# rednote-hilab/dots.ocr

Hardware: AMD Instinct MI355X
Metric: pages/sec, dots.ocr 1.7B bf16, A4@200dpi page batch (preprocess + ViT + prefill + 1024-token greedy decode + detokenise) (higher is better)
Workload: dtype bf16; 1 GPU; a4: 8 pages/GPU of 1654x2339 px -> 19824 patches, 5200 prompt tokens/page, max_new_tokens=1024, EOS disabled; pages_per_gpu=8, parallelism=dp1, decode_rows_in_flight=64

## Files before the change

dots_ocr_amd/csrc/engine.hip:

```cpp
#include <hip/hip_runtime.h>
#include <hip/hip_fp16.h>

#include <algorithm>
#include <cmath>
#include <cstdarg>
#include <cstddef>
#include <cstdio>
#include <cstdlib>
#include <cstring>
#include <string>
#include <unordered_map>
#include <vector>

#include "common.h"
#include "decode_layout.h"
#include "dots_ocr_hip.h"
#include "kernels.h"

namespace {

thread_local std::string g_create_error;

struct Tensor {
    bf16_t* p = nullptr;
// ... 1683 lines not shown
int dots_set_decode_plan(DotsEngine* e, int plan) {
    if (!e) return DOTS_E_INVALID;
    if (plan < 0 || plan > 5 || (plan & 6) == 6)
        return e->fail(DOTS_E_INVALID, "decode plan must be 0 (by stream) or 1 (partition plan on every step), + 2 (streaming attention) or + 4 (per-split attention)");
    const int part = plan & 1, stream = (plan & 2) ? 1 : (plan & 4) ? 0 : -1;
    if (part != e->force_part || stream != e->attn_stream) {
        e->force_part = part;
        e->attn_stream = stream;
        drop_step_graphs(e);
    }
    return DOTS_OK;
}

int dots_tower_tail(DotsEngine* e, int set, int* now) {
    if (!e) return DOTS_E_INVALID;
    if (set < -2 || set > e->cfg.v_layers) return e->fail(DOTS_E_INVALID, "tower tail must be -2 (query), -1 (adaptive) or 0 .. v_layers");
    if (set >= -1) e->tail_fixed = set;
    if (now) *now = e->tail_now;
    return DOTS_OK;
}

int dots_set_gemm_plan(DotsEngine* e, int plan) {
    if (!e) return DOTS_E_INVALID;
    if (plan < 0 || plan > 1) return e->fail(DOTS_E_INVALID, "gemm plan must be 0 (8-wave ping-pong) or 1 (one wave per SIMD)");
    gemm_set_plan(plan);
    return DOTS_OK;
}

int dots_get_logits(DotsEngine* e, float* out) {
    if (!e || !out) return DOTS_E_INVALID;
    if (e->B < 1) return e->fail(DOTS_E_STATE, "no prefilled batch");
    CK(hipSetDevice(e->device));
    CK(hipMemcpyAsync(out, e->d_logits, (size_t)e->B * e->cfg.vocab_size * 4, hipMemcpyDeviceToHost, e->stream));
    CK(hipStreamSynchronize(e->stream));
    return DOTS_OK;
}

int dots_set_next_tokens(DotsEngine* e, const int32_t* tokens, int B) {
    if (!e || !tokens || B != e->B) return e ? e->fail(DOTS_E_INVALID, "bad set_next_tokens arguments") : DOTS_E_INVALID;
    CK(hipSetDevice(e->device));
    CK(hipMemcpyAsync(e->cur_tokens, tokens, B * 4, hipMemcpyHostToDevice, e->stream));
    CK(hipStreamSynchronize(e->stream));
    return DOTS_OK;
}

int dots_get_last_tokens(DotsEngine* e, int32_t* out) {
    if (!e || !out) return DOTS_E_INVALID;
// ... 490 lines not shown
```

dots_ocr_amd/csrc/gemm.hip:

```cpp
#include <cstdlib>
#include <utility>

#include "common.h"
#include "kernels.h"

namespace {

constexpr int BM = 128, BN = 128, BK = 64;
constexpr int TILE_BYTES = 128 * 128;
#ifndef GEMM_GROUP_M
#define GEMM_GROUP_M 8
#endif
constexpr int GROUP_M = GEMM_GROUP_M;

DEVI float gelu_erf(float x) { return 0.5f * x * (1.0f + erff(x * 0.70710678118654752440f)); }
#ifdef GEMM_EXACT_SILU
DEVI float silu(float x) { return x / (1.0f + __expf(-x)); }
#else
DEVI float silu(float x) {
    const float d = 1.0f + __expf(fminf(-x, 80.f));
    const float r = __builtin_amdgcn_rcpf(d);
    const float q = x * r;
    return __builtin_fmaf(__builtin_fmaf(-q, d, x), r, q);
}
#endif

template <int EPI, int FN, int FM = 2>
DEVI void gemm_epilogue(const f32x16 (&acc)[FN][FM], const bf16_t* __restrict__ bias, const float* __restrict__ colscale, const bf16_t* R,
                        void* Cout, int M, int ldc, int nw0, int mw0, int l31, int hi, const float* __restrict__ rowscale = nullptr) {
#pragma unroll
    for (int fm = 0; fm < FM; ++fm) {
        const int m = mw0 + fm * 32 + l31;
        if (m >= M) continue;
        const float rs = rowscale ? rowscale[m] : 1.f;
        if constexpr (EPI == EPI_SWIGLU) {
            bf16_t* C = reinterpret_cast<bf16_t*>(Cout);
// ... 425 lines not shown
    const int gcol = SW ? ((l & 7) >> 2) * 64 + (l & 3) * 8 : (l & 15) * 8;
    u32x4 b0 = {0, 0, 0, 0}, b1 = {0, 0, 0, 0};
    f32x4 s00 = {1.f, 1.f, 1.f, 1.f}, s01 = s00, s10 = s00, s11 = s00;
    if (bias) {
        b0 = *reinterpret_cast<const u32x4*>(bias + nw0 + gcol);
        if (SW) b1 = *reinterpret_cast<const u32x4*>(bias + nw0 + gcol + 32);
    }
    if (colscale) {
        s00 = *reinterpret_cast<const f32x4*>(colscale + nw0 + gcol);
        s01 = *reinterpret_cast<const f32x4*>(colscale + nw0 + gcol + 4);
        if (SW) {
            s10 = *reinterpret_cast<const f32x4*>(colscale + nw0 + gcol + 32);
            s11 = *reinterpret_cast<const f32x4*>(colscale + nw0 + gcol + 36);
        }
    }
#pragma unroll
    for (int e = 0; e < 4; ++e) {
        cc.sc0[e] = s00[e]; cc.sc0[4 + e] = s01[e]; cc.sc1[e] = s10[e]; cc.sc1[4 + e] = s11[e];
        cc.bi0[2 * e] = lo_bf(b0[e]); cc.bi0[2 * e + 1] = hi_bf(b0[e]);
        cc.bi1[2 * e] = lo_bf(b1[e]); cc.bi1[2 * e + 1] = hi_bf(b1[e]);
    }
}

template <int EPI, bool FULL>
DEVI void w4_epilogue_lds(const f32x16 (&acc)[4][4], const W4Cols& cc, bool has_cols, const bf16_t* R,
                          bf16_t* __restrict__ C, int M, int ldc, int nw0, int mw0, int l, char* stage2) {
    const int hi = l >> 5, l31 = l & 31;
    constexpr bool SW = EPI == EPI_SWIGLU;
    constexpr int ITS = SW ? 4 : 8, RPI = SW ? 8 : 4;
    const int rrow = SW ? (l >> 3) : (l >> 4);
    const int gcol = SW ? ((l & 7) >> 2) * 64 + (l & 3) * 8 : (l & 15) * 8;
    const int col = SW ? nw0 / 2 + ((l & 7) >> 2) * 32 + (l & 3) * 8 : nw0 + gcol;
    u32x4 rr[2][8];
    auto load_r = [&](int fm, u32x4 (&dst)[8]) {
        if constexpr (EPI == EPI_RESIDUAL) {
#pragma unroll
            for (int it = 0; it < ITS; ++it) {
                const int m = FULL ? mw0 + fm * 32 + it * RPI + rrow : min(mw0 + fm * 32 + it * RPI + rrow, M - 1);
                dst[it] = *reinterpret_cast<const u32x4*>(R + (size_t)m * ldc + col);
            }
        }
    };
#ifdef W4_OLD_SWZ
    auto swz = [](int row) { return (row & 15) << 1; };
#else
    auto swz = [](int row) { return ((row & 15) << 1) ^ (row & 1) ^ ((row & 2) << 2); };
#endif
    const int wslot = swz(l31);
    char* const wrow = stage2 + l31 * 512;
#define W4_PUT(FM, IMG)                                                                                                   \
    _Pragma("unroll") for (int fn = 0; fn < 4; ++fn) _Pragma("unroll") for (int rq = 0; rq < 4; ++rq) {                     \
        const f32x4 v = {acc[fn][FM][4 * rq], acc[fn][FM][4 * rq + 1], acc[fn][FM][4 * rq + 2], acc[fn][FM][4 * rq + 3]};   \
        *reinterpret_cast<f32x4*>(wrow + (IMG) * 16384 + (((fn * 8 + rq * 2 + hi) ^ wslot) << 4)) = v;                      \
    }
    load_r(0, rr[0]);
    W4_PUT(0, 0)
#pragma unroll
    for (int fm = 0; fm < 4; ++fm) {
        if (fm + 1 < 4) {
            load_r(fm + 1, rr[(fm + 1) & 1]);
            if (fm == 0) { W4_PUT(1, 1) } else if (fm == 1) { W4_PUT(2, 0) } else { W4_PUT(3, 1) }
        }
        __builtin_amdgcn_sched_barrier(0);
        const char* img = stage2 + (fm & 1) * 16384;
        f32x4 a[ITS][SW ? 4 : 2];
#pragma unroll
        for (int it = 0; it < ITS; ++it) {
            const int row = it * RPI + rrow;
            const int sw = swz(row);
            const char* rp = img + row * 512;
            const int s0 = gcol >> 2;
            a[it][0] = *reinterpret_cast<const f32x4*>(rp + ((s0 ^ sw) << 4));
            a[it][1] = *reinterpret_cast<const f32x4*>(rp + (((s0 + 1) ^ sw) << 4));
            if constexpr (SW) {
                a[it][2] = *reinterpret_cast<const f32x4*>(rp + (((s0 + 8) ^ sw) << 4));
                a[it][3] = *reinterpret_cast<const f32x4*>(rp + (((s0 + 9) ^ sw) << 4));
            }
// ... 41 lines not shown

DEVI void w4_load_cols_rope(W4Cols& cc, const bf16_t* __restrict__ bias, const float* __restrict__ colscale, int nw0, int l) {
    const int gcol = (l & 15) * 8, pcol = gcol ^ 64;
    u32x4 b0 = {0, 0, 0, 0}, b1 = {0, 0, 0, 0};
    f32x4 s00 = {1.f, 1.f, 1.f, 1.f}, s01 = s00, s10 = s00, s11 = s00;
    if (bias) {
        b0 = *reinterpret_cast<const u32x4*>(bias + nw0 + gcol);
        b1 = *reinterpret_cast<const u32x4*>(bias + nw0 + pcol);
    }
    if (colscale) {
        s00 = *reinterpret_cast<const f32x4*>(colscale + nw0 + gcol);
        s01 = *reinterpret_cast<const f32x4*>(colscale + nw0 + gcol + 4);
        s10 = *reinterpret_cast<const f32x4*>(colscale + nw0 + pcol);
        s11 = *reinterpret_cast<const f32x4*>(colscale + nw0 + pcol + 4);
    }
#pragma unroll
    for (int e = 0; e < 4; ++e) {
        cc.sc0[e] = s00[e]; cc.sc0[4 + e] = s01[e]; cc.sc1[e] = s10[e]; cc.sc1[4 + e] = s11[e];
        cc.bi0[2 * e] = lo_bf(b0[e]); cc.bi0[2 * e + 1] = hi_bf(b0[e]);
        cc.bi1[2 * e] = lo_bf(b1[e]); cc.bi1[2 * e + 1] = hi_bf(b1[e]);
    }
}

template <bool FULL>
DEVI void w4_epilogue_qkrope(const f32x16 (&acc)[4][4], const W4Cols& cc, bool has_cols, const float2* __restrict__ cs, bf16_t* __restrict__ dst,
                             int M, int mw0, int l, char* stage2) {
    const int hi = l >> 5, l31 = l & 31;
    const int rrow = l >> 4, gcol = (l & 15) * 8;
    const bool lo_half = (l & 8) == 0;
    const float2* const tab = cs + (gcol & 63);
    auto swz = [](int row) { return ((row & 15) << 1) ^ (row & 1) ^ ((row & 2) << 2); };
    const int wslot = swz(l31);
    char* const wrow = stage2 + l31 * 512;
#define W4_PUT(FM, IMG)                                                                                                   \
    _Pragma("unroll") for (int fn = 0; fn < 4; ++fn) _Pragma("unroll") for (int rq = 0; rq < 4; ++rq) {                     \
        const f32x4 v = {acc[fn][FM][4 * rq], acc[fn][FM][4 * rq + 1], acc[fn][FM][4 * rq + 2], acc[fn][FM][4 * rq + 3]};   \
        *reinterpret_cast<f32x4*>(wrow + (IMG) * 16384 + (((fn * 8 + rq * 2 + hi) ^ wslot) << 4)) = v;                      \
    }
    f32x4 tb[2][2][4];
    auto load_t = [&](int qb, f32x4 (&d)[2][4]) {
#pragma unroll
        for (int it = 0; it < 2; ++it) {
            const int m = FULL ? mw0 + qb * 8 + it * 4 + rrow : min(mw0 + qb * 8 + it * 4 + rrow, M - 1);
            const f32x4* tp = reinterpret_cast<const f32x4*>(tab + (size_t)m * 64);
#pragma unroll
            for (int c = 0; c < 4; ++c) d[it][c] = tp[c];
        }
    };
    load_t(0, tb[0]);
    W4_PUT(0, 0)
#pragma unroll
    for (int qb = 0; qb < 16; ++qb) {
        const int fm = qb >> 2;
        if (qb + 1 < 16) load_t(qb + 1, tb[(qb + 1) & 1]);
        if ((qb & 3) == 0 && fm + 1 < 4) {
            if (fm == 0) { W4_PUT(1, 1) } else if (fm == 1) { W4_PUT(2, 0) } else { W4_PUT(3, 1) }
        }
        __builtin_amdgcn_sched_barrier(0);
        const char* img = stage2 + (fm & 1) * 16384;
        f32x4 a[2][4];
#pragma unroll
// ... 18 lines not shown
                for (int e = 0; e < 8; ++e) { o[e] = o[e] * cc.sc0[e] + cc.bi0[e]; u[e] = u[e] * cc.sc1[e] + cc.bi1[e]; }
            }
            uint32_t pk[4];
#pragma unroll
            for (int e = 0; e < 4; ++e) {
                const uint32_t ow = pack_bf2(o[2 * e], o[2 * e + 1]), uw = pack_bf2(u[2 * e], u[2 * e + 1]);
                const float x0 = lo_bf(ow), x1 = hi_bf(ow), y0 = lo_bf(uw), y1 = hi_bf(uw);
                const f32x4 t4 = tb[qb & 1][it][e];
                const float f0 = lo_half ? x0 : y0, g0 = lo_half ? t4[0] : t4[1], m0 = lo_half ? y0 : x0, n0_ = lo_half ? t4[1] : t4[0];
                const float p0 = m0 * n0_, p1 = y1 * t4[3];
                const float r0 = __builtin_fmaf(f0, g0, lo_half ? -p0 : p0), r1 = __builtin_fmaf(x1, t4[2], lo_half ? -p1 : p1);
                pk[e] = pack_bf2(r0, r1);
            }
            if (FULL || m < M) *reinterpret_cast<u32x4*>(dst + (size_t)m * 128 + gcol) = u32x4{pk[0], pk[1], pk[2], pk[3]};
        }
        __builtin_amdgcn_sched_barrier(0);
    }
#undef W4_PUT
}

template <int... I, class F> DEVI void gemm_static_for_impl(std::integer_sequence<int, I...>, F&& f) { (f(std::integral_constant<int, I>{}), ...); }
template <int N, class F> DEVI void gemm_static_for(F&& f) { gemm_static_for_impl(std::make_integer_sequence<int, N>{}, f); }

template <int EPI>
DEVI void gemm_bf16_w4_body(
    const bf16_t* __restrict__ A, const bf16_t* __restrict__ W, const bf16_t* __restrict__ bias,
    const float* __restrict__ colscale, const bf16_t* R, void* Cout, int M, int N, int K, int lda, int ldc, int m_tiles, int n_tiles, int group_m, const QkRope& rope) {
    extern __shared__ __attribute__((aligned(16))) char smem2[];
    (void)rope;

    const int tid = threadIdx.x;
    const int l = tid & 63;
    const int w = __builtin_amdgcn_readfirstlane(tid >> 6);
    const int hi = l >> 5, l31 = l & 31;

    int bid = xcd_remap(blockIdx.x, m_tiles * n_tiles);
    const int per_group = group_m * n_tiles;
    const int g = bid / per_group;
    const int first_m = g * group_m;
    const int gsz = min(m_tiles - first_m, group_m);
    const int in_grp = bid - g * per_group;
    const int tm = first_m + in_grp % gsz;
    const int tn = in_grp / gsz;
    const int m0 = tm * BM2, n0 = tn * BN2;

    const int prow = 8 * w + (l >> 3);
    const int chunk = ((l & 7) ^ ((4 * w + (l >> 4)) & 7)) << 4;
    const int w_src = prow * (K * 2) + chunk;
    int x_src[8];
#pragma unroll
    for (int i = 0; i < 8; ++i) x_src[i] = (min(m0 + prow + 32 * i, M - 1) - m0) * (lda * 2) + chunk;
    const __amdgpu_buffer_rsrc_t rw = __builtin_amdgcn_make_buffer_rsrc((void*)(W + (size_t)n0 * K), 0, 0x7ffffff0, 0x00020000);
    const __amdgpu_buffer_rsrc_t rx = __builtin_amdgcn_make_buffer_rsrc((void*)(A + (size_t)m0 * lda), 0, 0x7ffffff0, 0x00020000);
    const int w_step = 32 * K * 2;
    auto dma_w = [&](int t, int slot, int i) {
        __builtin_amdgcn_raw_ptr_buffer_load_lds(rw, (__attribute__((address_space(3))) void*)(smem2 + slot * W4_UNIT + (w + 4 * i) * 1024), 16, w_src,
                                                 t * 128 + i * w_step, 0, 0);
    };
    auto dma_x = [&](int t, int slot, int i) {
        __builtin_amdgcn_raw_ptr_buffer_load_lds(rx, (__attribute__((address_space(3))) void*)(smem2 + slot * W4_UNIT + (w + 4 * i) * 1024), 16, x_src[i],
                                                 t * 128, 0, 0);
    };

    const int wn = w >> 1, wm = w & 1;
    const int rsw = (l31 >> 1) & 7;
    const int lane_sw = ((hi ^ (rsw & 1)) << 4) | ((rsw >> 1) << 5);
    const int lds0 = (int)(uintptr_t)(__attribute__((address_space(3))) char*)smem2;
    const int a_lane = lds0 + (wn * 128 + l31) * 128 + lane_sw;
    const int b_lane = lds0 + (wm * 128 + l31) * 128 + lane_sw;
    auto frag = [&](int base, int ks, int f) {
        return *reinterpret_cast<const __attribute__((address_space(3))) bf16x8*>((uintptr_t)(uint32_t)((base ^ (ks << 5)) + f * 4096));
    };

#ifdef W4_PROF
    const unsigned long long pt0 = __builtin_amdgcn_s_memtime(), pw0 = wall_clock64();
#endif
    W4Cols cols;
    if constexpr (EPI == EPI_QKROPE) w4_load_cols_rope(cols, bias, colscale, n0 + wn * 128, l);
    else if constexpr (EPI != EPI_F32) w4_load_cols<EPI == EPI_SWIGLU>(cols, bias, colscale, n0 + wn * 128, l);

    f32x16 acc[4][4];
#pragma unroll
    for (int i = 0; i < 4; ++i)
#pragma unroll
        for (int j = 0; j < 4; ++j)
#pragma unroll
            for (int r = 0; r < 16; ++r) acc[i][j][r] = 0.f;

    const int nt = K / BK;
#ifdef W4_STAGGER
    if (blockIdx.x < 256) {
        const int naps = ((blockIdx.x >> 3) & 7) * nt * W4_STAGGER / 8;
        for (int i = 0; i < naps; ++i) __builtin_amdgcn_s_sleep(8);
    }
#endif
#pragma unroll
    for (int u = 0; u < 4; ++u)
#pragma unroll
        for (int i = 0; i < 8; ++i) {
            if (u & 1) dma_x(u >> 1, u, i);
            else dma_w(u >> 1, u, i);
        }
    asm volatile("s_waitcnt vmcnt(16)" ::: "memory");
    __builtin_amdgcn_s_barrier();
    bf16x8 fa[2][4], fb[2][4];
#pragma unroll
    for (int f = 0; f < 4; ++f) { fa[0][f] = frag(a_lane, 0, f); fb[0][f] = frag(b_lane + W4_UNIT, 0, f); }
#ifdef W4_PROF
    const unsigned long long pt1 = __builtin_amdgcn_s_memtime(), pw1 = wall_clock64();
#endif

    auto tile_body = [&](auto mode_c, int t, int u0) {
        constexpr int MODE = decltype(mode_c)::value;
        const int s1 = u0 + 1 >= W4_RING ? u0 + 1 - W4_RING : u0 + 1, s2 = u0 + 2 >= W4_RING ? u0 + 2 - W4_RING : u0 + 2;
        const int s3 = u0 + 3 >= W4_RING ? u0 + 3 - W4_RING : u0 + 3, s4 = u0 + 4 >= W4_RING ? u0 + 4 - W4_RING : u0 + 4;
        const int aw = a_lane + u0 * W4_UNIT, ax = b_lane + s1 * W4_UNIT;
        const int awn = a_lane + s2 * W4_UNIT, axn = b_lane + s3 * W4_UNIT;
        gemm_static_for<64>([&acc, &fa, &fb, &frag, &dma_w, &dma_x, aw, ax, awn, axn, t, u0, s4](auto gc) {
            constexpr int gp = decltype(gc)::value;
            (void)acc; (void)t; (void)u0; (void)s4; (void)dma_w; (void)dma_x;
            constexpr int ks = gp >> 4, idx = gp & 15, fn = idx >> 2, fm = idx & 3, cur = ks & 1;
            if constexpr (gp == 48 && MODE < 2) {
                if constexpr (MODE == 0) asm volatile("s_waitcnt vmcnt(8) lgkmcnt(0)" ::: "memory");
                else asm volatile("s_waitcnt vmcnt(0) lgkmcnt(0)" ::: "memory");
                __builtin_amdgcn_s_barrier();
            }
            if constexpr (idx < 8 && (ks < 3 || MODE < 2)) {
                constexpr int f = idx & 3;
                if constexpr (ks < 3) {
                    if constexpr (idx < 4) fa[cur ^ 1][f] = frag(aw, ks + 1, f);
                    else fb[cur ^ 1][f] = frag(ax, ks + 1, f);
                } else {
                    if constexpr (idx < 4) fa[cur ^ 1][f] = frag(awn, 0, f);
                    else fb[cur ^ 1][f] = frag(axn, 0, f);
                }
            }
#ifndef W4_NO_DMA
            if constexpr (MODE == 0) {
                if constexpr (gp == 8 || gp == 11 || gp == 14 || gp == 24 || gp == 27 || gp == 30 || gp == 40 || gp == 43) {
                    constexpr int i = gp < 16 ? (gp - 8) / 3 : gp < 32 ? 3 + (gp - 24) / 3 : 6 + (gp - 40) / 3;
                    dma_w(t + 2, s4, i);
                }
                if constexpr (gp >= 56) dma_x(t + 2, u0, gp - 56);
            }
#endif
            asm volatile("v_mfma_f32_32x32x16_bf16 %[d], %[a], %[b], %[d]" : [d] "+a"(acc[fn][fm]) : [a] "v"(fa[cur][fn]), [b] "v"(fb[cur][fm]));
        });
    };
    int u0 = 0;
    for (int t = 0; t < nt - 2; ++t) {
        tile_body(std::integral_constant<int, 0>{}, t, u0);
        u0 = u0 + 2 >= W4_RING ? u0 + 2 - W4_RING : u0 + 2;
    }
    tile_body(std::integral_constant<int, 1>{}, nt - 2, u0);
    u0 = u0 + 2 >= W4_RING ? u0 + 2 - W4_RING : u0 + 2;
    tile_body(std::integral_constant<int, 2>{}, nt - 1, u0);

#ifdef W4_PROF
    const unsigned long long pt2 = __builtin_amdgcn_s_memtime(), pw2 = wall_clock64();
#endif
    __syncthreads();
#ifdef W4_NO_STORE
#pragma unroll
    for (int i = 0; i < 4; ++i)
#pragma unroll
        for (int j = 0; j < 4; ++j) asm volatile("" ::"a"(acc[i][j]));
    return;
#endif
#ifdef W4_OLD_EPILOGUE
    if constexpr (EPI == EPI_F32 || EPI == EPI_SWIGLU) {
        gemm_epilogue<EPI, 4, 4>(acc, bias, colscale, R, Cout, M, ldc, n0 + wn * 128, m0 + wm * 128, l31, hi);
    } else {
        gemm_epilogue_lds<EPI, 4>(acc, bias, colscale, R, reinterpret_cast<bf16_t*>(Cout), M, ldc, n0 + wn * 128, m0 + wm * 128, l, smem2 + w * 16384);
    }
#else
    if constexpr (EPI == EPI_QKROPE) {
        const int head = (n0 + wn * 128) >> 7;
        const bool full = m0 + wm * 128 + 128 <= M, has_cols = bias != nullptr || colscale != nullptr;
        if (head < rope.n_rope_heads) {
            bf16_t* dst = head < rope.Hq ? rope.q + (size_t)head * rope.T * 128 : rope.k + (size_t)(head - rope.Hq) * rope.T * 128;
            if (full) w4_epilogue_qkrope<true>(acc, cols, has_cols, rope.cs, dst, M, m0 + wm * 128, l, smem2 + w * 32768);
            else w4_epilogue_qkrope<false>(acc, cols, has_cols, rope.cs, dst, M, m0 + wm * 128, l, smem2 + w * 32768);
        } else if (full) {
            w4_epilogue_lds<EPI_NONE, true>(acc, cols, has_cols, R, reinterpret_cast<bf16_t*>(Cout), M, ldc, n0 + wn * 128, m0 + wm * 128, l, smem2 + w * 32768);
        } else {
            w4_epilogue_lds<EPI_NONE, false>(acc, cols, has_cols, R, reinterpret_cast<bf16_t*>(Cout), M, ldc, n0 + wn * 128, m0 + wm * 128, l, smem2 + w * 32768);
        }
    } else if constexpr (EPI == EPI_F32) {
        gemm_epilogue<EPI, 4, 4>(acc, bias, colscale, R, Cout, M, ldc, n0 + wn * 128, m0 + wm * 128, l31, hi);
    } else if (m0 + wm * 128 + 128 <= M) {
        w4_epilogue_lds<EPI, true>(acc, cols, bias != nullptr || colscale != nullptr, R, reinterpret_cast<bf16_t*>(Cout), M, ldc, n0 + wn * 128, m0 + wm * 128, l, smem2 + w * 32768);
    } else {
        w4_epilogue_lds<EPI, false>(acc, cols, bias != nullptr || colscale != nullptr, R, reinterpret_cast<bf16_t*>(Cout), M, ldc, n0 + wn * 128, m0 + wm * 128, l, smem2 + w * 32768);
    }
#endif
#ifdef W4_PROF
    const unsigned long long pt2b = __builtin_amdgcn_s_memtime();
    asm volatile("s_waitcnt vmcnt(0)" ::: "memory");
    const unsigned long long pt3 = __builtin_amdgcn_s_memtime(), pw3 = wall_clock64();
    if ((blockIdx.x == 1000 || blockIdx.x == 2001 || blockIdx.x == 3002) && tid == 0)
        printf("W4_PROF epi %d N %d K %d blk %d: prologue %llu cyc / %.2f us, main loop %llu cyc / %.2f us (%.0f cyc per K tile), epilogue + drain %llu cyc / %.2f us; issue %llu drain %llu\n", EPI, N, K,
               (int)blockIdx.x, pt1 - pt0, (pw1 - pw0) * 0.01, pt2 - pt1, (pw2 - pw1) * 0.01, (double)(pt2 - pt1) / nt, pt3 - pt2, (pw3 - pw2) * 0.01, pt2b - pt2, pt3 - pt2b);
#endif
}

template <int EPI>
__global__ __launch_bounds__(256) void gemm_bf16_w4_kernel(
    const bf16_t* __restrict__ A, const bf16_t* __restrict__ W, const bf16_t* __restrict__ bias,
    const float* __restrict__ colscale, const bf16_t* R, void* Cout, int M, int N, int K, int lda, int ldc, int m_tiles, int n_tiles, int group_m) {
    gemm_bf16_w4_body<EPI>(A, W, bias, colscale, R, Cout, M, N, K, lda, ldc, m_tiles, n_tiles, group_m, QkRope{});
}
__global__ __launch_bounds__(256) void gemm_bf16_w4_qkrope_kernel(
    const bf16_t* __restrict__ A, const bf16_t* __restrict__ W, const bf16_t* __restrict__ bias,
    const float* __restrict__ colscale, void* Cout, int M, int N, int K, int lda, int ldc, int m_tiles, int n_tiles, int group_m, QkRope rope) {
    gemm_bf16_w4_body<EPI_QKROPE>(A, W, bias, colscale, nullptr, Cout, M, N, K, lda, ldc, m_tiles, n_tiles, group_m, rope);
}

typedef __attribute__((ext_vector_type(8))) int i32x8;

template <int EPI>
__global__ __launch_bounds__(512, 2) void gemm_fp8_256pp_kernel(
    const uint8_t* __restrict__ A, const float* __restrict__ rowscale, const uint8_t* __restrict__ W, const float* __restrict__ colscale,
    const bf16_t* __restrict__ bias, const bf16_t* R, void* Cout, int M, int N, int K, int ldc, int m_tiles, int n_tiles, int group_m) {
    extern __shared__ __attribute__((aligned(16))) char smem2[];
    constexpr int SUBK8 = 64;

    const int tid = threadIdx.x;
    const int l = tid & 63;
    const int w = __builtin_amdgcn_readfirstlane(tid >> 6);
    const int hi = l >> 5, l31 = l & 31;
    const int grp = w >> 2;

    int bid = xcd_remap(blockIdx.x, m_tiles * n_tiles);
    const int per_group = group_m * n_tiles;
    const int g = bid / per_group;
    const int first_m = g * group_m;
    const int gsz = min(m_tiles - first_m, group_m);
    const int in_grp = bid - g * per_group;
// ... 76 lines not shown
            acc[fn][1] = __builtin_amdgcn_mfma_scale_f32_32x32x64_f8f6f4(af[fn], bf_[1], acc[fn][1], 0, 0, 0, 0x7f7f7f7f, 0, 0x7f7f7f7f);
        }
        __builtin_amdgcn_s_setprio(0);
        __builtin_amdgcn_sched_barrier(0);
        if (grp == 0 || p + 1 < ns) __builtin_amdgcn_s_barrier();
        __builtin_amdgcn_sched_barrier(0);
    }
    if constexpr (EPI == EPI_SWIGLU) {
        gemm_epilogue<EPI, 4>(acc, bias, colscale, R, Cout, M, ldc, n0 + wn * 128, m0 + wm * 64, l31, hi, rowscale);
    } else {
        __syncthreads();
        gemm_epilogue_lds<EPI>(acc, bias, colscale, R, reinterpret_cast<bf16_t*>(Cout), M, ldc, n0 + wn * 128, m0 + wm * 64, l, smem2 + w * 16384, rowscale);
    }
}

}

static int raster_group_m(int row_bytes) {
    const int panel = 256 * row_bytes;
    return panel >= (4 << 20) ? 2 : panel >= (3 << 19) ? 4 : GROUP_M;
}

static int g_gemm_plan = -1;
int gemm_get_plan() {
    int p = __atomic_load_n(&g_gemm_plan, __ATOMIC_RELAXED);
    if (p < 0) {
        const char* ev = getenv("DOTS_OCR_GEMM_PLAN");
        p = ev ? (atoi(ev) != 0) : 1;
        __atomic_store_n(&g_gemm_plan, p, __ATOMIC_RELAXED);
    }
    return p;
}
void gemm_set_plan(int plan) { __atomic_store_n(&g_gemm_plan, plan != 0, __ATOMIC_RELAXED); }

template <int E>
static hipError_t launch_256(hipStream_t s, const bf16_t* A, const bf16_t* W, const bf16_t* bias, const float* colscale, const bf16_t* R, void* C,
                                int M, int N, int K, int lda, int ldc) {
    static uint32_t configured = 0;
    int dev = 0;
    hipError_t e = hipGetDevice(&dev);
    if (e != hipSuccess) return e;
    const uint32_t bit = 1u << (dev & 31);
    if (!(__atomic_load_n(&configured, __ATOMIC_ACQUIRE) & bit)) {
        e = hipFuncSetAttribute(reinterpret_cast<const void*>(&gemm_bf16_256_kernel<E>), hipFuncAttributeMaxDynamicSharedMemorySize, 2 * STAGE2);
        if (e != hipSuccess) return e;
        __atomic_fetch_or(&configured, bit, __ATOMIC_RELEASE);
    }
    const int m_tiles = (M + BM2 - 1) / BM2, n_tiles = N / BN2;
    static const bool lockstep = getenv("DOTS_OCR_GEMM_LOCKSTEP") != nullptr;
    if (lockstep || ldc % 8 != 0) {
        hipLaunchKernelGGL(gemm_bf16_256_kernel<E>, dim3(m_tiles * n_tiles), dim3(512), 2 * STAGE2, s, A, W, bias, colscale, R, C, M, N, K,
                           lda, ldc, m_tiles, n_tiles);
        return hipGetLastError();
    }
    if (gemm_get_plan() == 1 && K / BK >= 3) {
        static uint32_t configured_w4 = 0;
        if (!(__atomic_load_n(&configured_w4, __ATOMIC_ACQUIRE) & bit)) {
            e = hipFuncSetAttribute(reinterpret_cast<const void*>(&gemm_bf16_w4_kernel<E>), hipFuncAttributeMaxDynamicSharedMemorySize, W4_RING * W4_UNIT);
            if (e != hipSuccess) return e;
            __atomic_fetch_or(&configured_w4, bit, __ATOMIC_RELEASE);
        }
        hipLaunchKernelGGL(gemm_bf16_w4_kernel<E>, dim3(m_tiles * n_tiles), dim3(256), W4_RING * W4_UNIT, s, A, W, bias, colscale, R, C, M, N, K,
                           lda, ldc, m_tiles, n_tiles, raster_group_m(K * 2));
        return hipGetLastError();
    }
    static uint32_t configured_pp = 0;
    if (!(__atomic_load_n(&configured_pp, __ATOMIC_ACQUIRE) & bit)) {
        e = hipFuncSetAttribute(reinterpret_cast<const void*>(&gemm_bf16_256pp_kernel<E>), hipFuncAttributeMaxDynamicSharedMemorySize,
                                PP_STAGES * SUB_STAGE);
        if (e != hipSuccess) return e;
        __atomic_fetch_or(&configured_pp, bit, __ATOMIC_RELEASE);
    }
    hipLaunchKernelGGL(gemm_bf16_256pp_kernel<E>, dim3(m_tiles * n_tiles), dim3(512), PP_STAGES * SUB_STAGE, s, A, W, bias, colscale, R, C, M, N, K,
                       lda, ldc, m_tiles, n_tiles, raster_group_m(K * 2));
    return hipGetLastError();
}

hipError_t launch_gemm(hipStream_t s, const bf16_t* A, const bf16_t* W, const bf16_t* bias, const bf16_t* R,
                       void* C, int64_t M, int N, int K, int lda, int ldc, int epi, const float* colscale) {
    if (M <= 0) return hipSuccess;
    if (N % BN != 0 || K % BK != 0 || (lda % 8) != 0 || (ldc % 4) != 0) return hipErrorInvalidValue;
    static const bool force_small = getenv("DOTS_OCR_GEMM_128") != nullptr;
    if (N % BN2 == 0 && !force_small) {
        switch (epi) {
            case EPI_NONE: return launch_256<EPI_NONE>(s, A, W, bias, colscale, R, C, (int)M, N, K, lda, ldc);
// ... 5 lines not shown
        }
    }
    const int m_tiles = (int)((M + BM - 1) / BM), n_tiles = N / BN;
    dim3 grid(m_tiles * n_tiles), block(256);
#define LAUNCH(E)                                                                                       \
    hipLaunchKernelGGL(gemm_bf16_kernel<E>, grid, block, 0, s, A, W, bias, colscale, R, C, (int)M, N, K, lda, ldc, \
                       m_tiles, n_tiles)
    switch (epi) {
        case EPI_NONE: LAUNCH(EPI_NONE); break;
        case EPI_RESIDUAL: LAUNCH(EPI_RESIDUAL); break;
        case EPI_SWIGLU: LAUNCH(EPI_SWIGLU); break;
        case EPI_GELU: LAUNCH(EPI_GELU); break;
        case EPI_F32: LAUNCH(EPI_F32); break;
        default: return hipErrorInvalidValue;
    }
#undef LAUNCH
    return hipGetLastError();
}

hipError_t launch_gemm_qk_rope(hipStream_t s, const bf16_t* A, const bf16_t* W, const bf16_t* bias, bf16_t* qkv, int64_t M, int N, int K, int lda, int ldc,
                               const float2* cs, bf16_t* q, bf16_t* k, int Hq, int Hkv) {
    static const bool off = getenv("DOTS_OCR_QK_FUSE") && atoi(getenv("DOTS_OCR_QK_FUSE")) == 0;
    static const bool lockstep = getenv("DOTS_OCR_GEMM_LOCKSTEP") != nullptr, force_small = getenv("DOTS_OCR_GEMM_128") != nullptr;
    if (off || lockstep || force_small || gemm_get_plan() != 1 || N != (Hq + 2 * Hkv) * 128 || N % BN2 != 0 || K % BK != 0 || K / BK < 3 || lda % 8 != 0 || ldc % 8 != 0 ||
        !cs || !q || !k || M > 0x7fffffff)
        return hipErrorNotSupported;
    if (M <= 0) return hipSuccess;
    static uint32_t configured = 0;
    int dev = 0;
    hipError_t e = hipGetDevice(&dev);
    if (e != hipSuccess) return e;
    const uint32_t bit = 1u << (dev & 31);
    if (!(__atomic_load_n(&configured, __ATOMIC_ACQUIRE) & bit)) {
        e = hipFuncSetAttribute(reinterpret_cast<const void*>(&gemm_bf16_w4_qkrope_kernel), hipFuncAttributeMaxDynamicSharedMemorySize, W4_RING * W4_UNIT);
        if (e != hipSuccess) return e;
        __atomic_fetch_or(&configured, bit, __ATOMIC_RELEASE);
    }
    const int m_tiles = (int)((M + BM2 - 1) / BM2), n_tiles = N / BN2;
    const QkRope rope{cs, q, k, (long long)M, Hq, Hq + Hkv};
    hipLaunchKernelGGL(gemm_bf16_w4_qkrope_kernel, dim3(m_tiles * n_tiles), dim3(256), W4_RING * W4_UNIT, s, A, W, bias, (const float*)nullptr, (void*)qkv, (int)M, N, K,
                       lda, ldc, m_tiles, n_tiles, raster_group_m(K * 2), rope);
    return hipGetLastError();
}

bool gemm_fp8_supports(int N, int K) { return N % BN2 == 0 && K % 64 == 0; }

template <int E>
static hipError_t launch_fp8_t(hipStream_t s, const uint8_t* Aq, const float* rowscale, const uint8_t* Wq, const float* colscale, const bf16_t* bias,
                               const bf16_t* R, void* C, int M, int N, int K, int ldc) {
    static uint32_t configured = 0;
    int dev = 0;
    hipError_t e = hipGetDevice(&dev);
    if (e != hipSuccess) return e;
    const uint32_t bit = 1u << (dev & 31);
    if (!(__atomic_load_n(&configured, __ATOMIC_ACQUIRE) & bit)) {
        e = hipFuncSetAttribute(reinterpret_cast<const void*>(&gemm_fp8_256pp_kernel<E>), hipFuncAttributeMaxDynamicSharedMemorySize, PP_STAGES * SUB_STAGE);
        if (e != hipSuccess) return e;
        __atomic_fetch_or(&configured, bit, __ATOMIC_RELEASE);
    }
    const int m_tiles = (M + BM2 - 1) / BM2, n_tiles = N / BN2;
    hipLaunchKernelGGL(gemm_fp8_256pp_kernel<E>, dim3(m_tiles * n_tiles), dim3(512), PP_STAGES * SUB_STAGE, s, Aq, rowscale, Wq, colscale, bias, R, C, M, N, K,
                       ldc, m_tiles, n_tiles, raster_group_m(K));
    return hipGetLastError();
// ... 15 lines not shown
```

Before: 6.183 pages/s.

## Add GEMM plan 2 using 16x16x32 MFMAs and make it the default

Adds a variant of the one-wave-per-SIMD bf16 GEMM that computes its 128x128 per-wave tile with 8x8 v_mfma_f32_16x16x32_bf16 instructions instead of 4x4 32x32x16. LDS fragment addressing, swizzles, the fragment prefetch and DMA interleave schedule, and the LDS-staged, f32 and QK-rope epilogues are all reworked for the new accumulator layout. The default plan becomes 2. The aim is better MFMA throughput or issue behaviour for the ViT and prefill GEMMs, at the cost of more fragment loads and a new schedule whose interleaving may not hide memory latency as well.

```diff
diff --git a/dots_ocr_amd/csrc/engine.hip b/dots_ocr_amd/csrc/engine.hip
--- a/dots_ocr_amd/csrc/engine.hip
+++ b/dots_ocr_amd/csrc/engine.hip
@@ -1729,7 +1729,7 @@
 
 int dots_set_gemm_plan(DotsEngine* e, int plan) {
     if (!e) return DOTS_E_INVALID;
-    if (plan < 0 || plan > 1) return e->fail(DOTS_E_INVALID, "gemm plan must be 0 (8-wave ping-pong) or 1 (one wave per SIMD)");
+    if (plan < 0 || plan > 2) return e->fail(DOTS_E_INVALID, "gemm plan must be 0 (8-wave ping-pong), 1 (one wave per SIMD) or 2 (plan 1 on 16x16x32 MFMAs)");
     gemm_set_plan(plan);
     return DOTS_OK;
 }
diff --git a/dots_ocr_amd/csrc/gemm.hip b/dots_ocr_amd/csrc/gemm.hip
--- a/dots_ocr_amd/csrc/gemm.hip
+++ b/dots_ocr_amd/csrc/gemm.hip
@@ -1,4 +1,5 @@
 #include <cstdlib>
+#include <type_traits>
 #include <utility>
 
 #include "common.h"
@@ -12,6 +13,9 @@
 #define GEMM_GROUP_M 8
 #endif
 constexpr int GROUP_M = GEMM_GROUP_M;
+#ifndef GEMM_DEFAULT_PLAN
+#define GEMM_DEFAULT_PLAN 2
+#endif
 
 DEVI float gelu_erf(float x) { return 0.5f * x * (1.0f + erff(x * 0.70710678118654752440f)); }
 #ifdef GEMM_EXACT_SILU
@@ -483,9 +487,46 @@
     }
 }
 
-template <int EPI, bool FULL>
-DEVI void w4_epilogue_lds(const f32x16 (&acc)[4][4], const W4Cols& cc, bool has_cols, const bf16_t* R,
+template <int FM, class Swz>
+DEVI void w4_put16(const f32x4 (&acc)[8][8], Swz swz, char* img, int l) {
+    const int q = l >> 4, l15 = l & 15;
+#pragma unroll
+    for (int h = 0; h < 2; ++h) {
+        const int row = 16 * h + l15, wslot = swz(row);
+        char* const wrow = img + row * 512;
+#pragma unroll
+        for (int fn = 0; fn < 8; ++fn) *reinterpret_cast<f32x4*>(wrow + (((fn * 4 + q) ^ wslot) << 4)) = acc[fn][2 * FM + h];
+    }
+}
+
+DEVI void w4_epilogue_f32_m16(const f32x4 (&acc)[8][8], const bf16_t* __restrict__ bias, const float* __restrict__ colscale, float* __restrict__ C,
+                              int M, int ldc, int nw0, int mw0, int l) {
+#pragma unroll
+    for (int fm = 0; fm < 8; ++fm) {
+        const int m = mw0 + fm * 16 + (l & 15);
+        if (m >= M) continue;
+#pragma unroll
+        for (int fn = 0; fn < 8; ++fn) {
+            const int nb = nw0 + fn * 16 + 4 * (l >> 4);
+            f32x4 o = acc[fn][fm];
+            if (colscale) {
+                const f32x4 sc = *reinterpret_cast<const f32x4*>(colscale + nb);
+#pragma unroll
+                for (int e = 0; e < 4; ++e) o[e] *= sc[e];
+            }
+            if (bias) {
+                u32x2 bb = *reinterpret_cast<const u32x2*>(bias + nb);
+                o[0] += lo_bf(bb[0]); o[1] += hi_bf(bb[0]); o[2] += lo_bf(bb[1]); o[3] += hi_bf(bb[1]);
+            }
+            *reinterpret_cast<f32x4*>(C + (size_t)m * ldc + nb) = o;
+        }
+    }
+}
+
+template <int EPI, bool FULL, class Acc>
+DEVI void w4_epilogue_lds(const Acc& acc, const W4Cols& cc, bool has_cols, const bf16_t* R,
                           bf16_t* __restrict__ C, int M, int ldc, int nw0, int mw0, int l, char* stage2) {
+    constexpr bool M16 = std::is_same_v<Acc, f32x4[8][8]>;
     const int hi = l >> 5, l31 = l & 31;
     constexpr bool SW = EPI == EPI_SWIGLU;
     constexpr int ITS = SW ? 4 : 8, RPI = SW ? 8 : 4;
@@ -510,10 +551,11 @@
     const int wslot = swz(l31);
     char* const wrow = stage2 + l31 * 512;
 #define W4_PUT(FM, IMG)                                                                                                   \
+    if constexpr (M16) { w4_put16<FM>(acc, swz, stage2 + (IMG) * 16384, l); } else {                                       \
     _Pragma("unroll") for (int fn = 0; fn < 4; ++fn) _Pragma("unroll") for (int rq = 0; rq < 4; ++rq) {                     \
         const f32x4 v = {acc[fn][FM][4 * rq], acc[fn][FM][4 * rq + 1], acc[fn][FM][4 * rq + 2], acc[fn][FM][4 * rq + 3]};   \
         *reinterpret_cast<f32x4*>(wrow + (IMG) * 16384 + (((fn * 8 + rq * 2 + hi) ^ wslot) << 4)) = v;                      \
-    }
+    } }
     load_r(0, rr[0]);
     W4_PUT(0, 0)
 #pragma unroll
@@ -601,9 +643,10 @@
     }
 }
 
-template <bool FULL>
-DEVI void w4_epilogue_qkrope(const f32x16 (&acc)[4][4], const W4Cols& cc, bool has_cols, const float2* __restrict__ cs, bf16_t* __restrict__ dst,
+template <bool FULL, class Acc>
+DEVI void w4_epilogue_qkrope(const Acc& acc, const W4Cols& cc, bool has_cols, const float2* __restrict__ cs, bf16_t* __restrict__ dst,
                              int M, int mw0, int l, char* stage2) {
+    constexpr bool M16 = std::is_same_v<Acc, f32x4[8][8]>;
     const int hi = l >> 5, l31 = l & 31;
     const int rrow = l >> 4, gcol = (l & 15) * 8;
     const bool lo_half = (l & 8) == 0;
@@ -612,10 +655,11 @@
     const int wslot = swz(l31);
     char* const wrow = stage2 + l31 * 512;
 #define W4_PUT(FM, IMG)                                                                                                   \
+    if constexpr (M16) { w4_put16<FM>(acc, swz, stage2 + (IMG) * 16384, l); } else {                                       \
     _Pragma("unroll") for (int fn = 0; fn < 4; ++fn) _Pragma("unroll") for (int rq = 0; rq < 4; ++rq) {                     \
         const f32x4 v = {acc[fn][FM][4 * rq], acc[fn][FM][4 * rq + 1], acc[fn][FM][4 * rq + 2], acc[fn][FM][4 * rq + 3]};   \
         *reinterpret_cast<f32x4*>(wrow + (IMG) * 16384 + (((fn * 8 + rq * 2 + hi) ^ wslot) << 4)) = v;                      \
-    }
+    } }
     f32x4 tb[2][2][4];
     auto load_t = [&](int qb, f32x4 (&d)[2][4]) {
 #pragma unroll
@@ -680,7 +724,7 @@
 template <int... I, class F> DEVI void gemm_static_for_impl(std::integer_sequence<int, I...>, F&& f) { (f(std::integral_constant<int, I>{}), ...); }
 template <int N, class F> DEVI void gemm_static_for(F&& f) { gemm_static_for_impl(std::make_integer_sequence<int, N>{}, f); }
 
-template <int EPI>
+template <int EPI, bool M16 = false>
 DEVI void gemm_bf16_w4_body(
     const bf16_t* __restrict__ A, const bf16_t* __restrict__ W, const bf16_t* __restrict__ bias,
     const float* __restrict__ colscale, const bf16_t* R, void* Cout, int M, int N, int K, int lda, int ldc, int m_tiles, int n_tiles, int group_m, const QkRope& rope) {
@@ -721,13 +765,16 @@
     };
 
     const int wn = w >> 1, wm = w & 1;
-    const int rsw = (l31 >> 1) & 7;
-    const int lane_sw = ((hi ^ (rsw & 1)) << 4) | ((rsw >> 1) << 5);
+    constexpr int NF = M16 ? 8 : 4;
+    const int lrow = M16 ? (l & 15) : l31;
+    const int rsw = (lrow >> 1) & 7;
+    const int lane_sw = M16 ? (((l >> 4) ^ rsw) << 4) : (((hi ^ (rsw & 1)) << 4) | ((rsw >> 1) << 5));
     const int lds0 = (int)(uintptr_t)(__attribute__((address_space(3))) char*)smem2;
-    const int a_lane = lds0 + (wn * 128 + l31) * 128 + lane_sw;
-    const int b_lane = lds0 + (wm * 128 + l31) * 128 + lane_sw;
+    const int a_lane = lds0 + (wn * 128 + lrow) * 128 + lane_sw;
+    const int b_lane = lds0 + (wm * 128 + lrow) * 128 + lane_sw;
     auto frag = [&](int base, int ks, int f) {
-        return *reinterpret_cast<const __attribute__((address_space(3))) bf16x8*>((uintptr_t)(uint32_t)((base ^ (ks << 5)) + f * 4096));
+        return *reinterpret_cast<const __attribute__((address_space(3))) bf16x8*>(
+            (uintptr_t)(uint32_t)((base ^ (ks << (M16 ? 6 : 5))) + f * (M16 ? 2048 : 4096)));
     };
 
 #ifdef W4_PROF
@@ -737,13 +784,13 @@
     if constexpr (EPI == EPI_QKROPE) w4_load_cols_rope(cols, bias, colscale, n0 + wn * 128, l);
     else if constexpr (EPI != EPI_F32) w4_load_cols<EPI == EPI_SWIGLU>(cols, bias, colscale, n0 + wn * 128, l);
 
-    f32x16 acc[4][4];
-#pragma unroll
-    for (int i = 0; i < 4; ++i)
-#pragma unroll
-        for (int j = 0; j < 4; ++j)
-#pragma unroll
-            for (int r = 0; r < 16; ++r) acc[i][j][r] = 0.f;
+    std::conditional_t<M16, f32x4[8][8], f32x16[4][4]> acc;
+#pragma unroll
+    for (int i = 0; i < NF; ++i)
+#pragma unroll
+        for (int j = 0; j < NF; ++j)
+#pragma unroll
+            for (int r = 0; r < (M16 ? 4 : 16); ++r) acc[i][j][r] = 0.f;
 
     const int nt = K / BK;
 #ifdef W4_STAGGER
@@ -761,9 +808,9 @@
         }
     asm volatile("s_waitcnt vmcnt(16)" ::: "memory");
     __builtin_amdgcn_s_barrier();
-    bf16x8 fa[2][4], fb[2][4];
-#pragma unroll
-    for (int f = 0; f < 4; ++f) { fa[0][f] = frag(a_lane, 0, f); fb[0][f] = frag(b_lane + W4_UNIT, 0, f); }
+    bf16x8 fa[2][NF], fb[2][NF];
+#pragma unroll
+    for (int f = 0; f < NF; ++f) { fa[0][f] = frag(a_lane, 0, f); fb[0][f] = frag(b_lane + W4_UNIT, 0, f); }
 #ifdef W4_PROF
     const unsigned long long pt1 = __builtin_amdgcn_s_memtime(), pw1 = wall_clock64();
 #endif
@@ -805,14 +852,50 @@
             asm volatile("v_mfma_f32_32x32x16_bf16 %[d], %[a], %[b], %[d]" : [d] "+a"(acc[fn][fm]) : [a] "v"(fa[cur][fn]), [b] "v"(fb[cur][fm]));
         });
     };
+    auto tile_body16 = [&](auto mode_c, int t, int u0) {
+        constexpr int MODE = decltype(mode_c)::value;
+        const int s1 = u0 + 1 >= W4_RING ? u0 + 1 - W4_RING : u0 + 1, s2 = u0 + 2 >= W4_RING ? u0 + 2 - W4_RING : u0 + 2;
+        const int s3 = u0 + 3 >= W4_RING ? u0 + 3 - W4_RING : u0 + 3, s4 = u0 + 4 >= W4_RING ? u0 + 4 - W4_RING : u0 + 4;
+        const int aw = a_lane + u0 * W4_UNIT, ax = b_lane + s1 * W4_UNIT;
+        const int awn = a_lane + s2 * W4_UNIT, axn = b_lane + s3 * W4_UNIT;
+        gemm_static_for<128>([&acc, &fa, &fb, &frag, &dma_w, &dma_x, aw, ax, awn, axn, t, u0, s4](auto gc) {
+            constexpr int gp = decltype(gc)::value;
+            (void)acc; (void)t; (void)u0; (void)s4; (void)dma_w; (void)dma_x; (void)awn; (void)axn;
+            constexpr int ks = gp >> 6, idx = gp & 63, fn = idx >> 3, fm = idx & 7;
+            if constexpr (gp == 96 && MODE < 2) {
+                if constexpr (MODE == 0) asm volatile("s_waitcnt vmcnt(8) lgkmcnt(0)" ::: "memory");
+                else asm volatile("s_waitcnt vmcnt(0) lgkmcnt(0)" ::: "memory");
+                __builtin_amdgcn_s_barrier();
+            }
+            constexpr bool rd1 = ks == 0 && idx < 16, rd0 = gp >= 96 && (gp & 1) == 0 && MODE < 2;
+            if constexpr (rd1 || rd0) {
+                constexpr int j = rd1 ? idx : (gp - 96) >> 1, set = rd1 ? 1 : 0;
+                const int bw = rd1 ? aw : awn, bx = rd1 ? ax : axn;
+                if constexpr (j == 0) fa[set][0] = frag(bw, set, 0);
+                else if constexpr (j <= 8) fb[set][j - 1] = frag(bx, set, j - 1);
+                else fa[set][j - 8] = frag(bw, set, j - 8);
+            }
+#ifndef W4_NO_DMA
+            if constexpr (MODE == 0) {
+                if constexpr (gp >= 20 && gp <= 90 && (gp - 20) % 10 == 0) dma_w(t + 2, s4, (gp - 20) / 10);
+                if constexpr (gp >= 97 && (gp - 97) % 4 == 0) dma_x(t + 2, u0, (gp - 97) / 4);
+            }
+#endif
+            asm volatile("v_mfma_f32_16x16x32_bf16 %[d], %[a], %[b], %[d]" : [d] "+a"(acc[fn][fm]) : [a] "v"(fa[ks][fn]), [b] "v"(fb[ks][fm]));
+        });
+    };
+    auto run_tile = [&](auto mode_c, int t, int u0) {
+        if constexpr (M16) tile_body16(mode_c, t, u0);
+        else tile_body(mode_c, t, u0);
+    };
     int u0 = 0;
     for (int t = 0; t < nt - 2; ++t) {
-        tile_body(std::integral_constant<int, 0>{}, t, u0);
+        run_tile(std::integral_constant<int, 0>{}, t, u0);
         u0 = u0 + 2 >= W4_RING ? u0 + 2 - W4_RING : u0 + 2;
     }
-    tile_body(std::integral_constant<int, 1>{}, nt - 2, u0);
+    run_tile(std::integral_constant<int, 1>{}, nt - 2, u0);
     u0 = u0 + 2 >= W4_RING ? u0 + 2 - W4_RING : u0 + 2;
-    tile_body(std::integral_constant<int, 2>{}, nt - 1, u0);
+    run_tile(std::integral_constant<int, 2>{}, nt - 1, u0);
 
 #ifdef W4_PROF
     const unsigned long long pt2 = __builtin_amdgcn_s_memtime(), pw2 = wall_clock64();
@@ -820,18 +903,20 @@
     __syncthreads();
 #ifdef W4_NO_STORE
 #pragma unroll
-    for (int i = 0; i < 4; ++i)
-#pragma unroll
-        for (int j = 0; j < 4; ++j) asm volatile("" ::"a"(acc[i][j]));
+    for (int i = 0; i < NF; ++i)
+#pragma unroll
+        for (int j = 0; j < NF; ++j) asm volatile("" ::"a"(acc[i][j]));
     return;
 #endif
 #ifdef W4_OLD_EPILOGUE
-    if constexpr (EPI == EPI_F32 || EPI == EPI_SWIGLU) {
-        gemm_epilogue<EPI, 4, 4>(acc, bias, colscale, R, Cout, M, ldc, n0 + wn * 128, m0 + wm * 128, l31, hi);
-    } else {
-        gemm_epilogue_lds<EPI, 4>(acc, bias, colscale, R, reinterpret_cast<bf16_t*>(Cout), M, ldc, n0 + wn * 128, m0 + wm * 128, l, smem2 + w * 16384);
-    }
-#else
+    if constexpr (!M16) {
+        if constexpr (EPI == EPI_F32 || EPI == EPI_SWIGLU) {
+            gemm_epilogue<EPI, 4, 4>(acc, bias, colscale, R, Cout, M, ldc, n0 + wn * 128, m0 + wm * 128, l31, hi);
+        } else {
+            gemm_epilogue_lds<EPI, 4>(acc, bias, colscale, R, reinterpret_cast<bf16_t*>(Cout), M, ldc, n0 + wn * 128, m0 + wm * 128, l, smem2 + w * 16384);
+        }
+    } else
+#endif
     if constexpr (EPI == EPI_QKROPE) {
         const int head = (n0 + wn * 128) >> 7;
         const bool full = m0 + wm * 128 + 128 <= M, has_cols = bias != nullptr || colscale != nullptr;
@@ -845,19 +930,19 @@
             w4_epilogue_lds<EPI_NONE, false>(acc, cols, has_cols, R, reinterpret_cast<bf16_t*>(Cout), M, ldc, n0 + wn * 128, m0 + wm * 128, l, smem2 + w * 32768);
         }
     } else if constexpr (EPI == EPI_F32) {
-        gemm_epilogue<EPI, 4, 4>(acc, bias, colscale, R, Cout, M, ldc, n0 + wn * 128, m0 + wm * 128, l31, hi);
+        if constexpr (M16) w4_epilogue_f32_m16(acc, bias, colscale, reinterpret_cast<float*>(Cout), M, ldc, n0 + wn * 128, m0 + wm * 128, l);
+        else gemm_epilogue<EPI, 4, 4>(acc, bias, colscale, R, Cout, M, ldc, n0 + wn * 128, m0 + wm * 128, l31, hi);
     } else if (m0 + wm * 128 + 128 <= M) {
         w4_epilogue_lds<EPI, true>(acc, cols, bias != nullptr || colscale != nullptr, R, reinterpret_cast<bf16_t*>(Cout), M, ldc, n0 + wn * 128, m0 + wm * 128, l, smem2 + w * 32768);
     } else {
         w4_epilogue_lds<EPI, false>(acc, cols, bias != nullptr || colscale != nullptr, R, reinterpret_cast<bf16_t*>(Cout), M, ldc, n0 + wn * 128, m0 + wm * 128, l, smem2 + w * 32768);
     }
-#endif
 #ifdef W4_PROF
     const unsigned long long pt2b = __builtin_amdgcn_s_memtime();
     asm volatile("s_waitcnt vmcnt(0)" ::: "memory");
     const unsigned long long pt3 = __builtin_amdgcn_s_memtime(), pw3 = wall_clock64();
     if ((blockIdx.x == 1000 || blockIdx.x == 2001 || blockIdx.x == 3002) && tid == 0)
-        printf("W4_PROF epi %d N %d K %d blk %d: prologue %llu cyc / %.2f us, main loop %llu cyc / %.2f us (%.0f cyc per K tile), epilogue + drain %llu cyc / %.2f us; issue %llu drain %llu\n", EPI, N, K,
+        printf("W4_PROF m16 %d epi %d N %d K %d blk %d: prologue %llu cyc / %.2f us, main loop %llu cyc / %.2f us (%.0f cyc per K tile), epilogue + drain %llu cyc / %.2f us; issue %llu drain %llu\n", (int)M16, EPI, N, K,
                (int)blockIdx.x, pt1 - pt0, (pw1 - pw0) * 0.01, pt2 - pt1, (pw2 - pw1) * 0.01, (double)(pt2 - pt1) / nt, pt3 - pt2, (pw3 - pw2) * 0.01, pt2b - pt2, pt3 - pt2b);
 #endif
 }
@@ -872,6 +957,17 @@
     const bf16_t* __restrict__ A, const bf16_t* __restrict__ W, const bf16_t* __restrict__ bias,
     const float* __restrict__ colscale, void* Cout, int M, int N, int K, int lda, int ldc, int m_tiles, int n_tiles, int group_m, QkRope rope) {
     gemm_bf16_w4_body<EPI_QKROPE>(A, W, bias, colscale, nullptr, Cout, M, N, K, lda, ldc, m_tiles, n_tiles, group_m, rope);
+}
+template <int EPI>
+__global__ __launch_bounds__(256) void gemm_bf16_w4m16_kernel(
+    const bf16_t* __restrict__ A, const bf16_t* __restrict__ W, const bf16_t* __restrict__ bias,
+    const float* __restrict__ colscale, const bf16_t* R, void* Cout, int M, int N, int K, int lda, int ldc, int m_tiles, int n_tiles, int group_m) {
+    gemm_bf16_w4_body<EPI, true>(A, W, bias, colscale, R, Cout, M, N, K, lda, ldc, m_tiles, n_tiles, group_m, QkRope{});
+}
+__global__ __launch_bounds__(256) void gemm_bf16_w4m16_qkrope_kernel(
+    const bf16_t* __restrict__ A, const bf16_t* __restrict__ W, const bf16_t* __restrict__ bias,
+    const float* __restrict__ colscale, void* Cout, int M, int N, int K, int lda, int ldc, int m_tiles, int n_tiles, int group_m, QkRope rope) {
+    gemm_bf16_w4_body<EPI_QKROPE, true>(A, W, bias, colscale, nullptr, Cout, M, N, K, lda, ldc, m_tiles, n_tiles, group_m, rope);
 }
 
 typedef __attribute__((ext_vector_type(8))) int i32x8;
@@ -994,16 +1090,25 @@
 }
 
 static int g_gemm_plan = -1;
+static int gemm_plan_of(int v) { return v == 2 ? 2 : v != 0; }
 int gemm_get_plan() {
     int p = __atomic_load_n(&g_gemm_plan, __ATOMIC_RELAXED);
     if (p < 0) {
         const char* ev = getenv("DOTS_OCR_GEMM_PLAN");
-        p = ev ? (atoi(ev) != 0) : 1;
+        p = ev ? gemm_plan_of(atoi(ev)) : GEMM_DEFAULT_PLAN;
         __atomic_store_n(&g_gemm_plan, p, __ATOMIC_RELAXED);
     }
     return p;
 }
-void gemm_set_plan(int plan) { __atomic_store_n(&g_gemm_plan, plan != 0, __ATOMIC_RELAXED); }
+void gemm_set_plan(int plan) { __atomic_store_n(&g_gemm_plan, gemm_plan_of(plan), __ATOMIC_RELAXED); }
+
+template <class F>
+static hipError_t w4_configure(F* kernel, uint32_t& configured, uint32_t bit) {
+    if (__atomic_load_n(&configured, __ATOMIC_ACQUIRE) & bit) return hipSuccess;
+    const hipError_t e = hipFuncSetAttribute(reinterpret_cast<const void*>(kernel), hipFuncAttributeMaxDynamicSharedMemorySize, W4_RING * W4_UNIT);
+    if (e == hipSuccess) __atomic_fetch_or(&configured, bit, __ATOMIC_RELEASE);
+    return e;
+}
 
 template <int E>
 static hipError_t launch_256(hipStream_t s, const bf16_t* A, const bf16_t* W, const bf16_t* bias, const float* colscale, const bf16_t* R, void* C,
@@ -1025,14 +1130,13 @@
                            lda, ldc, m_tiles, n_tiles);
         return hipGetLastError();
     }
-    if (gemm_get_plan() == 1 && K / BK >= 3) {
-        static uint32_t configured_w4 = 0;
-        if (!(__atomic_load_n(&configured_w4, __ATOMIC_ACQUIRE) & bit)) {
-            e = hipFuncSetAttribute(reinterpret_cast<const void*>(&gemm_bf16_w4_kernel<E>), hipFuncAttributeMaxDynamicSharedMemorySize, W4_RING * W4_UNIT);
-            if (e != hipSuccess) return e;
-            __atomic_fetch_or(&configured_w4, bit, __ATOMIC_RELEASE);
-        }
-        hipLaunchKernelGGL(gemm_bf16_w4_kernel<E>, dim3(m_tiles * n_tiles), dim3(256), W4_RING * W4_UNIT, s, A, W, bias, colscale, R, C, M, N, K,
+    const int plan = gemm_get_plan();
+    if (plan >= 1 && K / BK >= 3) {
+        static uint32_t configured_w4 = 0, configured_m16 = 0;
+        auto* kernel = plan == 2 ? &gemm_bf16_w4m16_kernel<E> : &gemm_bf16_w4_kernel<E>;
+        e = w4_configure(kernel, plan == 2 ? configured_m16 : configured_w4, bit);
+        if (e != hipSuccess) return e;
+        hipLaunchKernelGGL(kernel, dim3(m_tiles * n_tiles), dim3(256), W4_RING * W4_UNIT, s, A, W, bias, colscale, R, C, M, N, K,
                            lda, ldc, m_tiles, n_tiles, raster_group_m(K * 2));
         return hipGetLastError();
     }
@@ -1084,23 +1188,22 @@
                                const float2* cs, bf16_t* q, bf16_t* k, int Hq, int Hkv) {
     static const bool off = getenv("DOTS_OCR_QK_FUSE") && atoi(getenv("DOTS_OCR_QK_FUSE")) == 0;
     static const bool lockstep = getenv("DOTS_OCR_GEMM_LOCKSTEP") != nullptr, force_small = getenv("DOTS_OCR_GEMM_128") != nullptr;
-    if (off || lockstep || force_small || gemm_get_plan() != 1 || N != (Hq + 2 * Hkv) * 128 || N % BN2 != 0 || K % BK != 0 || K / BK < 3 || lda % 8 != 0 || ldc % 8 != 0 ||
+    const int plan = gemm_get_plan();
+    if (off || lockstep || force_small || plan == 0 || N != (Hq + 2 * Hkv) * 128 || N % BN2 != 0 || K % BK != 0 || K / BK < 3 || lda % 8 != 0 || ldc % 8 != 0 ||
         !cs || !q || !k || M > 0x7fffffff)
         return hipErrorNotSupported;
     if (M <= 0) return hipSuccess;
-    static uint32_t configured = 0;
+    static uint32_t configured = 0, configured_m16 = 0;
     int dev = 0;
     hipError_t e = hipGetDevice(&dev);
     if (e != hipSuccess) return e;
     const uint32_t bit = 1u << (dev & 31);
-    if (!(__atomic_load_n(&configured, __ATOMIC_ACQUIRE) & bit)) {
-        e = hipFuncSetAttribute(reinterpret_cast<const void*>(&gemm_bf16_w4_qkrope_kernel), hipFuncAttributeMaxDynamicSharedMemorySize, W4_RING * W4_UNIT);
-        if (e != hipSuccess) return e;
-        __atomic_fetch_or(&configured, bit, __ATOMIC_RELEASE);
-    }
+    auto* kernel = plan == 2 ? &gemm_bf16_w4m16_qkrope_kernel : &gemm_bf16_w4_qkrope_kernel;
+    e = w4_configure(kernel, plan == 2 ? configured_m16 : configured, bit);
+    if (e != hipSuccess) return e;
     const int m_tiles = (int)((M + BM2 - 1) / BM2), n_tiles = N / BN2;
     const QkRope rope{cs, q, k, (long long)M, Hq, Hq + Hkv};
-    hipLaunchKernelGGL(gemm_bf16_w4_qkrope_kernel, dim3(m_tiles * n_tiles), dim3(256), W4_RING * W4_UNIT, s, A, W, bias, (const float*)nullptr, (void*)qkv, (int)M, N, K,
+    hipLaunchKernelGGL(kernel, dim3(m_tiles * n_tiles), dim3(256), W4_RING * W4_UNIT, s, A, W, bias, (const float*)nullptr, (void*)qkv, (int)M, N, K,
                        lda, ldc, m_tiles, n_tiles, raster_group_m(K * 2), rope);
     return hipGetLastError();
 }
```

Result: no change. 6.213 pages/s, median of 6 (+0.5%).
